# FebriantiW/Homomorphic-Encryption-and-Federated-Learning-based-Privacy-Preserving-CNN-Training-

Measured on AMD Instinct MI355X. Metric: fl_rounds_per_sec, higher is better.
Workload: dtype bf16; 1 GPU; model=cnn2, image=28x28x1, global_batch=32, local_epochs=10, samples_per_client=720, augment=none, parallelism=fl-dp1 (1 GPU = 1 client), device=cuda

## Files before the change

### hefl/csrc/bindings.cpp

```cpp
#include <torch/extension.h>

#include <vector>

void ntt_batch(torch::Tensor x, torch::Tensor w, torch::Tensor wsh, int64_t q);
void intt_batch(torch::Tensor x, torch::Tensor winv, torch::Tensor winvsh,
                int64_t q, int64_t ninv, int64_t ninvsh);
torch::Tensor modmul(torch::Tensor a, torch::Tensor b, int64_t q);
torch::Tensor modmul_scalar(torch::Tensor a, int64_t s, int64_t q);
torch::Tensor modadd(torch::Tensor a, torch::Tensor b, int64_t q);
torch::Tensor modsub(torch::Tensor a, torch::Tensor b, int64_t q);
void modreduce_(torch::Tensor x, torch::Tensor qs);
torch::Tensor cbd21(torch::Tensor bits);
void ntt_limbs(torch::Tensor x, torch::Tensor w, torch::Tensor wsh,
               torch::Tensor qs, int64_t L);
void intt_limbs(torch::Tensor x, torch::Tensor winv, torch::Tensor winvsh,
                torch::Tensor qs, torch::Tensor ninv, torch::Tensor ninvsh,
                int64_t L);
torch::Tensor modmul_limbs(torch::Tensor a, torch::Tensor b, torch::Tensor qs,
                           torch::Tensor ratios, int64_t L, int64_t n);
torch::Tensor modmul_scalar_limbs(torch::Tensor a, torch::Tensor scalars,
                                  torch::Tensor shoups, torch::Tensor qs,
                                  int64_t L, int64_t n);
torch::Tensor modadd_limbs(torch::Tensor a, torch::Tensor b, torch::Tensor qs,
                           int64_t L, int64_t n);
torch::Tensor modadd3_limbs(torch::Tensor a, torch::Tensor b, torch::Tensor c,
                            torch::Tensor qs, int64_t L, int64_t n);
torch::Tensor modsub_limbs(torch::Tensor a, torch::Tensor b, torch::Tensor qs,
                           int64_t L, int64_t aL, int64_t n);
torch::Tensor bcast_center_mod(torch::Tensor x, int64_t qc, torch::Tensor qs,
                               torch::Tensor ratios, int64_t L);
std::vector<torch::Tensor> ct_mul(torch::Tensor a, torch::Tensor b,
                                  torch::Tensor qs, torch::Tensor ratios,
                                  int64_t L, int64_t n);
std::vector<torch::Tensor> ks_inner(torch::Tensor dig, torch::Tensor rlk,
                                    torch::Tensor qs, torch::Tensor ratios,
                                    int64_t D, int64_t Lp, int64_t n);
torch::Tensor uniform_center_rns(torch::Tensor bits, int64_t smudge_bits,
                                 torch::Tensor qs, torch::Tensor ratios,
                                 int64_t L);
torch::Tensor pdec_share(torch::Tensor ct, torch::Tensor s_hat,
                         torch::Tensor e_hat, bool add_c0, torch::Tensor qs,
                         torch::Tensor ratios);
torch::Tensor galois_lift(torch::Tensor c, int64_t ginv, torch::Tensor qs,
                          torch::Tensor ratios);
torch::Tensor galois_perm_add(torch::Tensor ct, torch::Tensor ks0,
                              torch::Tensor ks1, torch::Tensor perm,
                              torch::Tensor qs);

torch::Tensor fft_encode(torch::Tensor vals, torch::Tensor tw_enc,
                         double scale);
torch::Tensor fft_decode(torch::Tensor coeffs, torch::Tensor tw_dec,
                         double scale, int64_t k);

torch::Tensor conv2d_fwd(torch::Tensor x, torch::Tensor w, torch::Tensor b,
                         int64_t stride, bool relu, int64_t pad);
torch::Tensor conv2d_dgrad(torch::Tensor dy, torch::Tensor w, int64_t stride,
                           int64_t H, int64_t W, int64_t pad);
torch::Tensor conv2d_wgrad(torch::Tensor dy, torch::Tensor x, int64_t stride,
                           int64_t R, int64_t S, int64_t pad, int64_t gkey);
torch::Tensor linear_fwd(torch::Tensor x, torch::Tensor w, torch::Tensor b,
                         bool relu);
torch::Tensor linear_dgrad(torch::Tensor dy, torch::Tensor w);
torch::Tensor linear_wgrad(torch::Tensor dy, torch::Tensor x);
std::vector<torch::Tensor> maxpool2x2_fwd(torch::Tensor x);
torch::Tensor synth_batch(torch::Tensor templates, torch::Tensor labels,
                          int64_t seed, double zoom, double shear,
                          int64_t flip);
torch::Tensor synth_batch_g(torch::Tensor templates, torch::Tensor labels,
                            torch::Tensor seed_buf, int64_t salt, double zoom,
                            double shear, int64_t flip);
torch::Tensor maxpool2x2_bwd(torch::Tensor dy, torch::Tensor idx, int64_t H,
                             int64_t W);
std::vector<torch::Tensor> softmax_xent_fwd(torch::Tensor logits,
                                            torch::Tensor labels,
                                            torch::Tensor acc_loss,
                                            torch::Tensor acc_correct);
torch::Tensor softmax_xent_bwd(torch::Tensor probs, torch::Tensor labels,
                               torch::Tensor dloss, bool out_bf16);
void fused_adam(torch::Tensor p, torch::Tensor g, torch::Tensor m,
                torch::Tensor v, double lr, double b1, double b2, double eps,
                double bc1, double bc2);
void adam_prep(torch::Tensor step, torch::Tensor sched, torch::Tensor hyper,
               double b1, double b2);
torch::Tensor relu_bwd(torch::Tensor dy, torch::Tensor y);
std::vector<torch::Tensor> bn_fwd(torch::Tensor x, torch::Tensor gamma,
                                  torch::Tensor beta, torch::Tensor rmean,
                                  torch::Tensor rvar, double eps,
                                  double momentum, bool relu,
                                  torch::Tensor sums);
torch::Tensor bn_apply(torch::Tensor x, torch::Tensor mean,
                       torch::Tensor invstd, torch::Tensor gamma,
                       torch::Tensor beta, bool relu);
std::vector<torch::Tensor> bn_bwd(torch::Tensor dy, torch::Tensor x,
                                  torch::Tensor mean, torch::Tensor invstd,
                                  torch::Tensor gamma, bool train,
                                  torch::Tensor relu_y, torch::Tensor fwd_sums);
std::vector<torch::Tensor> maxpool_fwd(torch::Tensor x, int64_t k, int64_t s,
// ... 51 lines not shown
    m.def("cbd21", &cbd21, "centered binomial eta=21 from 64-bit draws");
    m.def("ntt_limbs", &ntt_limbs, "fused multi-limb forward NTT [R, L, n]");
    m.def("intt_limbs", &intt_limbs, "fused multi-limb inverse NTT");
    m.def("modmul_limbs", &modmul_limbs);
    m.def("modmul_scalar_limbs", &modmul_scalar_limbs);
    m.def("modadd_limbs", &modadd_limbs, "per-limb modular add over [.., L, n]");
    m.def("modadd3_limbs", &modadd3_limbs, "fused 3-way per-limb modular add");
    m.def("modsub_limbs", &modsub_limbs, "per-limb modular sub over [.., L, n]");
    m.def("bcast_center_mod", &bcast_center_mod,
          "[.., n] -> [.., L, n] center + per-limb Barrett reduce");
    m.def("ct_mul", &ct_mul, "fused ct x ct tensor product (d0, d1, d2)");
    m.def("ks_inner", &ks_inner, "fused key-switch digit inner product");
    m.def("uniform_center_rns", &uniform_center_rns,
          "64-bit draws [.., n] -> smudging noise residues [.., L, n]");
    m.def("pdec_share", &pdec_share,
          "threshold decryption share c1*s + e (+ c0) over [.., 2, L, n]");
    m.def("galois_lift", &galois_lift,
          "X -> X^g on key-switch digits [.., D, n], lifted to [.., D, Lp, n]");
    m.def("galois_perm_add", &galois_perm_add,
          "rotated ciphertext (c0[perm] + ks0, ks1) over [.., 2, L, n]");
    m.def("fft_encode", &fft_encode,
          "CKKS special-FFT encode: f64 slots -> int64 coeffs");
    m.def("fft_decode", &fft_decode,
          "CKKS special-FFT decode: int64 coeffs -> f32 slots");
    m.def("conv2d_fwd", &conv2d_fwd);
    m.def("conv2d_dgrad", &conv2d_dgrad);
    m.def("conv2d_wgrad", &conv2d_wgrad, py::arg("dy"), py::arg("x"),
          py::arg("stride"), py::arg("R"), py::arg("S"), py::arg("pad"),
          py::arg("gkey") = 0);
    m.def("linear_fwd", &linear_fwd);
    m.def("linear_dgrad", &linear_dgrad);
    m.def("linear_wgrad", &linear_wgrad);
    m.def("maxpool2x2_fwd", &maxpool2x2_fwd);
    m.def("synth_batch", &synth_batch, py::arg("templates"), py::arg("labels"),
          py::arg("seed"), py::arg("zoom") = 0.0, py::arg("shear") = 0.0,
          py::arg("flip") = 0);
    m.def("synth_batch_g", &synth_batch_g, py::arg("templates"),
          py::arg("labels"), py::arg("seed_buf"), py::arg("salt"),
          py::arg("zoom") = 0.0, py::arg("shear") = 0.0, py::arg("flip") = 0);
    m.def("maxpool2x2_bwd", &maxpool2x2_bwd);
    m.def("softmax_xent_fwd", &softmax_xent_fwd);
    m.def("softmax_xent_bwd", &softmax_xent_bwd);
    m.def("fused_adam", &fused_adam);
    m.def("adam_prep", &adam_prep);
    m.def("relu_bwd", &relu_bwd);
    m.def("bn_fwd", &bn_fwd);
    m.def("bn_apply", &bn_apply);
    m.def("bn_bwd", &bn_bwd);
    m.def("maxpool_fwd", &maxpool_fwd);
    m.def("maxpool_bwd", &maxpool_bwd);
    m.def("avgpool_global_fwd", &avgpool_global_fwd);
    m.def("avgpool_global_bwd", &avgpool_global_bwd);
    m.def("add_relu", &add_relu);
    m.def("bias_grad", &bias_grad, py::arg("dy"), py::arg("gkey") = 0);
    m.def("relu_bias_bwd", &relu_bias_bwd, py::arg("dy"), py::arg("y"),
          py::arg("gkey") = 0);
    m.def("pool_relu_bias_bwd", &pool_relu_bias_bwd, py::arg("dy"),
          py::arg("idx"), py::arg("p"), py::arg("H"), py::arg("W"),
          py::arg("gkey") = 0);
    m.def("fused_adam_mt", &fused_adam_mt);
    m.def("pad_channels", &pad_channels,
          "zero-pad NHWC channel dim to C8 (stem -> glds MFMA path)");
    m.def("dense_head2_fwd", &dense_head2_fwd);
    m.def("dense_head2_bwd", &dense_head2_bwd,
          "single-launch backward of the 2-layer dense head (M <= 32)");
    m.def("linear_bwd_pair", &linear_bwd_pair,
// ... 10 lines not shown
```

### hefl/csrc/cnn.hip

```cpp

#include <hip/hip_runtime.h>
#include <hip/hip_bf16.h>
#include <torch/extension.h>
#include <ATen/cuda/CUDAContext.h>

#include <algorithm>
#include <unordered_map>

#define CHECK_GPU(x) TORCH_CHECK((x).is_cuda(), #x " must be on GPU")

namespace {

using bf16_t = __bf16;
typedef bf16_t bf16x8 __attribute__((ext_vector_type(8)));
typedef float f32x4 __attribute__((ext_vector_type(4)));
typedef unsigned short u16x8 __attribute__((ext_vector_type(8)));

__device__ __forceinline__ float bf2f(unsigned short u) {
    union { unsigned int i; float f; } v;
    v.i = ((unsigned int)u) << 16;
    return v.f;
}

__device__ __forceinline__ unsigned short f2bf(float f) {
    union { float f; unsigned int i; } v;
    v.f = f;
    unsigned int x = v.i;
    unsigned int lsb = (x >> 16) & 1;
    x += 0x7fffu + lsb;
    if ((v.i & 0x7fffffffu) > 0x7f800000u) return 0x7fc0u;
    return (unsigned short)(x >> 16);
}


constexpr int BM = 64;
constexpr int BN = 16;
constexpr int BK = 32;
constexpr int TPB = 256;

// ... 128 lines not shown

template <int BM, int BN, int WM, int WN, int FM, int FN>
__device__ __forceinline__ void tile_mfma(
    const unsigned short (&As)[BM][32], const unsigned short (&Bs)[BN][32],
    f32x4 (&acc)[FM][FN], int wave, int lane) {
    const int wm = wave / WN, wn = wave % WN;
    const int half = lane >> 4, sub = lane & 15;
    bf16x8 a[FM], b[FN];
#pragma unroll
    for (int i = 0; i < FM; ++i)
        a[i] = *reinterpret_cast<const bf16x8*>(
            &As[wm * FM * 16 + i * 16 + sub][half * 8]);
#pragma unroll
    for (int j = 0; j < FN; ++j)
        b[j] = *reinterpret_cast<const bf16x8*>(
            &Bs[wn * FN * 16 + j * 16 + sub][half * 8]);
#pragma unroll
    for (int i = 0; i < FM; ++i)
#pragma unroll
        for (int j = 0; j < FN; ++j)
            acc[i][j] = __builtin_amdgcn_mfma_f32_16x16x32_bf16(a[i], b[j],
                                                                acc[i][j], 0, 0, 0);
}

__device__ __forceinline__ void copy16(unsigned short* dst,
                                       const unsigned short* src) {
    *reinterpret_cast<uint4*>(dst) = *reinterpret_cast<const uint4*>(src);
}

__device__ __forceinline__ void zero16(unsigned short* dst) {
    *reinterpret_cast<uint4*>(dst) = uint4{0, 0, 0, 0};
}

template <int BM, int BN, int WM, int WN, int FM, int FN>
__global__ void __launch_bounds__(TPB)
conv_fwd_kernel(const unsigned short* __restrict__ x,
                const unsigned short* __restrict__ w,
                const float* __restrict__ bias, unsigned short* __restrict__ y,
                ConvShape s, int relu) {
    __shared__ ConvTile<BM, BN, WM, WN, FM, FN> sm;
    constexpr int RPT = BM * 4 / TPB;
    const int tid = threadIdx.x;
    const int wave = tid >> 6;
    const int lane = tid & 63;
    const int m0 = blockIdx.x * BM;
    const int n0 = blockIdx.y * BN;
    const int M = s.N * s.OH * s.OW;
    const int KK = s.R * s.S * s.C;
    const bool fast = (s.C % 8 == 0);

    int arows[RPT], am_[RPT], a_n[RPT], a_oh[RPT], a_ow[RPT];
    const int akc = (tid & 3) * 8;
#pragma unroll
    for (int t = 0; t < RPT; ++t) {
        arows[t] = (tid + t * TPB) >> 2;
        const int am = m0 + arows[t];
        am_[t] = am;
        a_n[t] = a_oh[t] = a_ow[t] = 0;
        if (am < M) {
            a_n[t] = am / (s.OH * s.OW);
            int rem = am % (s.OH * s.OW);
            a_oh[t] = rem / s.OW;
            a_ow[t] = rem % s.OW;
        }
    }

    f32x4 acc[FM][FN];
#pragma unroll
    for (int i = 0; i < FM; ++i)
#pragma unroll
        for (int j = 0; j < FN; ++j) acc[i][j] = f32x4{0.f, 0.f, 0.f, 0.f};

    for (int k0 = 0; k0 < KK; k0 += 32) {
#pragma unroll
        for (int t = 0; t < RPT; ++t) {
            const int k = k0 + akc;
            unsigned short* dst = &sm.As[arows[t]][akc];
            if (am_[t] < M && k < KK) {
                if (fast) {
                    int rs = (int)fdiv((unsigned)k, s.fC), c = k - rs * s.C;
                    int r = (int)fdiv((unsigned)rs, s.fS), ss = rs - r * s.S;
                    int ih = a_oh[t] * s.stride + r - s.pad;
                    int iw = a_ow[t] * s.stride + ss - s.pad;
                    if (ih >= 0 && ih < s.H && iw >= 0 && iw < s.W)
                        copy16(dst, x + ((((int64_t)a_n[t] * s.H + ih) * s.W + iw)
                                             * s.C + c));
                    else
                        zero16(dst);
                } else {
#pragma unroll
                    for (int j = 0; j < 8; ++j) {
                        int kk = k + j;
                        unsigned short v = 0;
                        if (kk < KK) {
                            int rs = (int)fdiv((unsigned)kk, s.fC);
                            int c = kk - rs * s.C;
// ... 8 lines not shown
                    }
                }
            } else {
                zero16(dst);
            }
        }
        for (int i = tid; i < BN * 4; i += TPB) {
            const int col = i >> 2;
            const int kc = (i & 3) * 8;
            const int ko = n0 + col, k = k0 + kc;
            unsigned short* dst = &sm.Bs[col][kc];
            if (ko < s.Kout && k < KK) {
                if ((KK & 7) == 0) {
                    copy16(dst, w + (int64_t)ko * KK + k);
                } else {
#pragma unroll
                    for (int j = 0; j < 8; ++j)
                        dst[j] = (k + j < KK) ? w[(int64_t)ko * KK + k + j] : 0;
                }
            } else {
                zero16(dst);
            }
        }
        __syncthreads();
        tile_mfma<BM, BN, WM, WN, FM, FN>(sm.As, sm.Bs, acc, wave, lane);
        __syncthreads();
    }
    const int wm = wave / WN, wn = wave % WN;
#pragma unroll
    for (int j = 0; j < FN; ++j) {
        const int col = n0 + wn * FN * 16 + j * 16 + (lane & 15);
        if (col >= s.Kout) continue;
        const float bv = bias ? bias[col] : 0.f;
#pragma unroll
        for (int i = 0; i < FM; ++i)
#pragma unroll
            for (int r = 0; r < 4; ++r) {
                int row = m0 + wm * FM * 16 + i * 16 + (lane >> 4) * 4 + r;
                if (row >= M) continue;
                float v = acc[i][j][r] + bv;
                if (relu) v = v > 0.f ? v : 0.f;
                y[(int64_t)row * s.Kout + col] = f2bf(v);
            }
    }
}


typedef uint32_t __attribute__((address_space(3))) lds_u32_t;
typedef const uint32_t __attribute__((address_space(1))) glb_u32_t;

__device__ __forceinline__ int xcd_remap(int wg, int nwg) {
    if (nwg < 16) return wg;
    const int xcd = wg & 7;
    const int q = nwg >> 3, r = nwg & 7;
    const int base = xcd < r ? xcd * (q + 1) : r * (q + 1) + (xcd - r) * q;
    return base + (wg >> 3);
}

__device__ __forceinline__ void glds16(const unsigned short* src, void* lds_base) {
    __builtin_amdgcn_global_load_lds((glb_u32_t*)src, (lds_u32_t*)lds_base, 16,
                                     0, 0);
}

template <int BM, int BN, int WM, int WN, int FM, int FN, int BK = 32>
__global__ void __launch_bounds__(TPB)
conv_fwd_glds_kernel(const unsigned short* __restrict__ x,
                     const unsigned short* __restrict__ w,
                     const float* __restrict__ bias,
                     unsigned short* __restrict__ y,
                     float* __restrict__ y32,
                     const unsigned short* __restrict__ zbuf, ConvShape s,
                     int relu, int k_chunks) {
    __shared__ unsigned short smem[3 * (BM + BN) * BK];
    auto As = [&](int buf) -> unsigned short (*)[BK] {
        return reinterpret_cast<unsigned short(*)[BK]>(smem + buf * (BM + BN) * BK);
    };
    auto Bs = [&](int buf) -> unsigned short (*)[BK] {
        return reinterpret_cast<unsigned short(*)[BK]>(smem + buf * (BM + BN) * BK
                                                       + BM * BK);
    };
    constexpr int RPT = BM * (BK / 8) / TPB;
    constexpr int BPT = BN * (BK / 8) / TPB;
    const int tid = threadIdx.x;
    const int wave = tid >> 6;
    const int lane = tid & 63;
    const int m0 = xcd_remap(blockIdx.x, gridDim.x) * BM;
    const int n0 = blockIdx.y * BN;
    const int M = s.N * s.OH * s.OW;
    const int KK = s.R * s.S * s.C;

    constexpr int CPR = BK / 8;
    int a_n[RPT], a_oh[RPT], a_ow[RPT];
    int akcs[RPT], arow3[RPT];
    bool a_ok[RPT];
#pragma unroll
    for (int t = 0; t < RPT; ++t) {
        const int arow = (tid + t * TPB) / CPR;
        arow3[t] = (arow >> 2) & 3;
        akcs[t] = ((tid % CPR) ^ (CPR == 4 ? arow3[t] : 0)) * 8;
        const int am = m0 + arow;
        a_ok[t] = am < M;
        a_n[t] = a_oh[t] = a_ow[t] = 0;
        if (a_ok[t]) {
            a_n[t] = am / (s.OH * s.OW);
            int rem = am % (s.OH * s.OW);
            a_oh[t] = rem / s.OW;
            a_ow[t] = rem % s.OW;
        }
    }

    auto stage = [&](int buf, int k0) {
#pragma unroll
        for (int t = 0; t < RPT; ++t) {
            const int k = k0 + akcs[t];
            const unsigned short* src = zbuf;
            if (a_ok[t] && k < KK) {
                int rs = (int)fdiv((unsigned)k, s.fC), c = k - rs * s.C;
                int r = (int)fdiv((unsigned)rs, s.fS), ss = rs - r * s.S;
                int ih = a_oh[t] * s.stride + r - s.pad;
                int iw = a_ow[t] * s.stride + ss - s.pad;
                if (ih >= 0 && ih < s.H && iw >= 0 && iw < s.W)
                    src = x + ((((int64_t)a_n[t] * s.H + ih) * s.W + iw) * s.C
                               + c);
            }
            char* base = (char*)&As(buf)[0][0] + (wave + t * 4) * 1024;
            glds16(src, base);
        }
#pragma unroll
        for (int t = 0; t < BPT; ++t) {
            const int i = tid + t * TPB;
            const int korow = i / CPR;
            const int ko = n0 + korow;
            const int kc = ((i % CPR) ^ (CPR == 4 ? ((korow >> 2) & 3) : 0)) * 8;
            const int k = k0 + kc;
            const unsigned short* src = zbuf;
            if (ko < s.Kout && k < KK) src = w + (int64_t)ko * KK + k;
            char* base = (char*)&Bs(buf)[0][0] + (wave + t * 4) * 1024;
            glds16(src, base);
        }
    };
// ... 22 lines not shown
            const int wm = wave / WN, wn = wave % WN;
            const int half = lane >> 4, sub = lane & 15;
            const int swz = (BK == 32) ? ((sub >> 2) & 3) : 0;
#pragma unroll
            for (int kk = 0; kk < BK; kk += 32) {
                bf16x8 a[FM], b[FN];
#pragma unroll
                for (int i = 0; i < FM; ++i)
                    a[i] = *reinterpret_cast<const bf16x8*>(
                        &As(buf)[wm * FM * 16 + i * 16 + sub]
                                [kk + ((half ^ swz) * 8)]);
#pragma unroll
                for (int j = 0; j < FN; ++j)
                    b[j] = *reinterpret_cast<const bf16x8*>(
                        &Bs(buf)[wn * FN * 16 + j * 16 + sub]
                                [kk + ((half ^ swz) * 8)]);
#pragma unroll
                for (int i = 0; i < FM; ++i)
#pragma unroll
                    for (int j = 0; j < FN; ++j)
                        acc[i][j] = __builtin_amdgcn_mfma_f32_16x16x32_bf16(
                            a[i], b[j], acc[i][j], 0, 0, 0);
            }
        }
        buf = buf == 2 ? 0 : buf + 1;
    }
    asm volatile("s_waitcnt vmcnt(0)" ::: "memory");
    const int wm = wave / WN, wn = wave % WN;
#pragma unroll
    for (int j = 0; j < FN; ++j) {
        const int col = n0 + wn * FN * 16 + j * 16 + (lane & 15);
        if (col >= s.Kout) continue;
        const float bv = bias ? bias[col] : 0.f;
#pragma unroll
        for (int i = 0; i < FM; ++i)
#pragma unroll
            for (int r = 0; r < 4; ++r) {
                int row = m0 + wm * FM * 16 + i * 16 + (lane >> 4) * 4 + r;
                if (row >= M) continue;
                if (k_chunks > 1) {
                    atomicAdd(y32 + (int64_t)row * s.Kout + col, acc[i][j][r]);
                } else {
                    float v = acc[i][j][r] + bv;
                    if (relu) v = v > 0.f ? v : 0.f;
                    y[(int64_t)row * s.Kout + col] = f2bf(v);
                }
            }
    }
}


__device__ __forceinline__ int swz128(int byte_off) {
    return byte_off ^ (((byte_off >> 9) & 1) << 5);
}

template <int BM, int BN, int WM, int WN, int FM, int FN, bool PAD0>
__global__ void __launch_bounds__(TPB)
conv_fwd_glds64_kernel(const unsigned short* __restrict__ x,
                       const unsigned short* __restrict__ w,
                       const float* __restrict__ bias,
                       unsigned short* __restrict__ y,
                       float* __restrict__ y32,
                       const unsigned short* __restrict__ zbuf, ConvShape s,
                       int relu, int k_chunks) {
    constexpr int BK = 64;
    constexpr int NW = TPB / 64;
    static_assert(WM * WN == NW, "wave grid must cover the block");
    static_assert(BM == WM * FM * 16 && BN == WN * FN * 16, "tile mismatch");
    constexpr int ABYTES = BM * BK * 2;
    constexpr int RPT = (BM * BK / 8) / TPB;
    constexpr int BPT = (BN * BK / 8) / TPB;
    static_assert(RPT * TPB * 8 == BM * BK && BPT * TPB * 8 == BN * BK);
    __shared__ unsigned short smem[2 * (BM + BN) * BK];
    const int tid = threadIdx.x;
    const int wave = tid >> 6;
    const int lane = tid & 63;
    const int m0 = blockIdx.x * BM;
    const int n0 = blockIdx.y * BN;
    const int M = s.N * s.OH * s.OW;
    const int KK = s.R * s.S * s.C;
// ... 2938 lines not shown
        }
        (void)hipMemsetAsync(p, 0, numel * sizeof(float), stream);
        it = bufs.emplace(key, std::make_pair(p, numel)).first;
    }
    if (it->second.second != numel) {
        ok = false;
        return {};
    }
    ok = true;
    return torch::from_blob(it->second.first, sizes,
                            opts.dtype(torch::kFloat32));
}

float* acc_pool(int64_t n, const torch::TensorOptions& opts,
                hipStream_t stream, torch::Tensor& holder) {
    static torch::Tensor pool;
    auto f32 = opts.dtype(torch::kFloat32);
    if (!pool.defined() || pool.device() != f32.device_opt().value() ||
        pool.numel() < n) {
        hipStreamCaptureStatus st = hipStreamCaptureStatusNone;
        (void)hipStreamIsCapturing(stream, &st);
        if (st != hipStreamCaptureStatusNone) {
            holder = torch::zeros({n}, f32);
            return holder.data_ptr<float>();
        }
        pool = torch::zeros({n}, f32);
    }
    return pool.data_ptr<float>();
}

}


torch::Tensor conv2d_fwd(torch::Tensor x, torch::Tensor w, torch::Tensor b,
                         int64_t stride, bool relu, int64_t pad) {
    CHECK_GPU(x);
    TORCH_CHECK(x.is_contiguous() && w.is_contiguous());
    TORCH_CHECK(x.dtype() == torch::kBFloat16 && w.dtype() == torch::kBFloat16);
    ConvShape s = make_shape(x, w, (int)stride, (int)pad);
    auto y = torch::empty({s.N, s.OH, s.OW, s.Kout}, x.options());
    const int M = s.N * s.OH * s.OW;
    const float* bias = b.numel() ? b.data_ptr<float>() : nullptr;
    auto stream = at::cuda::getCurrentCUDAStream();
    const int KKf = s.R * s.S * s.C;
    const char* t3env = getenv("HEFL_TILE3");
    const int t3mode = t3env ? t3env[0] - '0' : 1;
    if (t3mode != 0 && s.R == 3 && s.S == 3 && s.stride == 1 && s.pad <= 1 &&
        s.C % 32 == 0 && s.Kout > 16 &&
        (t3mode >= 2 || s.Kout <= 32)) {
        const int BN3 = (t3mode == 3 || s.Kout <= 32) ? 32 : 64;
        const int kt = ceildiv(s.Kout, BN3);
        const int64_t min_tiles = t3mode == 2 ? 1 : 256;
        auto tiles = [&](int th, int tw) {
            return (int64_t)s.N * ceildiv(s.OH, th) * ceildiv(s.OW, tw) * kt;
        };
        int TH = 0;
        if (s.OH >= 12 && tiles(16, 16) >= min_tiles) TH = 16;
        else if (t3mode >= 2 && s.OH >= 6 && tiles(8, 16) >= min_tiles) TH = 8;
        if (TH) {
            const int th_ = ceildiv(s.OH, TH), tw_ = ceildiv(s.OW, 16);
            dim3 grid((unsigned)(s.N * th_ * tw_), (unsigned)kt);
            #define LAUNCH_T3(TH_, TW_, BN_, WM_, WN_, FM_, FN_)              \
                hipLaunchKernelGGL(                                           \
                    (conv_fwd_tile3_kernel<TH_, TW_, BN_, WM_, WN_, FM_,      \
                                           FN_>),                             \
                    grid, dim3(TPB), 0, stream, bf_ptr(x), bf_ptr(w), bias,   \
                    bf_ptr_mut(y), s, relu ? 1 : 0, th_, tw_)
            if (TH == 16 && BN3 == 64)      LAUNCH_T3(16, 16, 64, 2, 2, 8, 2);
            else if (TH == 16)              LAUNCH_T3(16, 16, 32, 4, 1, 4, 2);
            else if (BN3 == 64)             LAUNCH_T3(8, 16, 64, 2, 2, 4, 2);
            else                            LAUNCH_T3(8, 16, 32, 2, 2, 4, 1);
            #undef LAUNCH_T3
            return y;
        }
    }
    static const bool use64 = [] {
        const char* e = getenv("HEFL_GLDS64");
        return e && e[0] == '1';
    }();
    if (use64 && s.Kout > 16 && s.C % 8 == 0 && KKf % 8 == 0) {
        static torch::Tensor zbuf64;
        if (!zbuf64.defined() || zbuf64.device() != x.device())
            zbuf64 = torch::zeros({8}, x.options());
        const bool narrow = s.Kout <= 32;
        const int BM = narrow ? 256 : 128, BN = narrow ? 32 : 64;
        int tiles = ceildiv(M, BM) * ceildiv(s.Kout, BN);
        int ksteps = ceildiv(KKf, 64);
        int k_chunks = 1;
        if (tiles < 256 && ksteps >= 8)
            k_chunks = std::max(1, std::min(ksteps / 2, 512 / std::max(tiles, 1)));
        dim3 grid(ceildiv(M, BM), ceildiv(s.Kout, BN), k_chunks);
        torch::Tensor y32;
        float* y32p = nullptr;
        if (k_chunks > 1)
            y32p = acc_pool((int64_t)M * s.Kout, x.options(), stream, y32);
        #define LAUNCH_F64(BM_, BN_, WM_, WN_, FM_, FN_, P0)                  \
            hipLaunchKernelGGL((conv_fwd_glds64_kernel<BM_, BN_, WM_, WN_,    \
                                                       FM_, FN_, P0>),       \
                               grid, dim3(TPB), 0, stream, bf_ptr(x),         \
                               bf_ptr(w), bias, bf_ptr_mut(y), y32p,          \
                               bf_ptr(zbuf64), s, relu ? 1 : 0, k_chunks)
        if (narrow) {
            if (s.pad == 0) LAUNCH_F64(256, 32, 4, 1, 4, 2, true);
            else            LAUNCH_F64(256, 32, 4, 1, 4, 2, false);
        } else {
            if (s.pad == 0) LAUNCH_F64(128, 64, 2, 2, 4, 2, true);
            else            LAUNCH_F64(128, 64, 2, 2, 4, 2, false);
        }
        #undef LAUNCH_F64
        if (k_chunks > 1) {
            int64_t total = (int64_t)M * s.Kout;
            hipLaunchKernelGGL(linear_epilogue_kernel,
                               dim3((int)std::min<int64_t>(ceildiv(total, 256), 2048)),
                               dim3(256), 0, stream, y32p, bias,
                               bf_ptr_mut(y), total, s.Kout, relu ? 1 : 0, 1, 1);
        }
        return y;
    }
    if (s.Kout > 16 && s.C % 8 == 0 && KKf % 8 == 0) {
        static torch::Tensor zbuf;
        if (!zbuf.defined() || zbuf.device() != x.device())
            zbuf = torch::zeros({8}, x.options());
        int tiles = ceildiv(M, 64) * ceildiv(s.Kout, 64);
        int ksteps = ceildiv(KKf, 32);
        int k_chunks = 1;
        if (tiles < 256 && ksteps >= 16)
            k_chunks = std::max(1, std::min(ksteps / 4, 512 / tiles));
        dim3 grid(ceildiv(M, 64), ceildiv(s.Kout, 64), k_chunks);
        if (k_chunks > 1) {
            torch::Tensor y32h;
            float* y32p = acc_pool((int64_t)M * s.Kout, x.options(), stream,
                                   y32h);
            hipLaunchKernelGGL((conv_fwd_glds_kernel<64, 64, 2, 2, 2, 2, 32>),
                               grid, dim3(TPB), 0, stream, bf_ptr(x), bf_ptr(w),
                               bias, bf_ptr_mut(y), y32p,
                               bf_ptr(zbuf), s, relu ? 1 : 0, k_chunks);
            int64_t total = (int64_t)M * s.Kout;
            hipLaunchKernelGGL(linear_epilogue_kernel,
                               dim3((int)std::min<int64_t>(ceildiv(total, 256), 2048)),
                               dim3(256), 0, stream, y32p, bias,
                               bf_ptr_mut(y), total, s.Kout, relu ? 1 : 0, 1, 1);
        } else {
            hipLaunchKernelGGL((conv_fwd_glds_kernel<64, 64, 2, 2, 2, 2, 32>),
                               grid, dim3(TPB), 0, stream, bf_ptr(x), bf_ptr(w),
                               bias, bf_ptr_mut(y), (float*)nullptr,
                               bf_ptr(zbuf), s, relu ? 1 : 0, 1);
        }
    } else if (s.Kout > 16) {
        dim3 grid(ceildiv(M, 64), ceildiv(s.Kout, 64));
        hipLaunchKernelGGL((conv_fwd_kernel<64, 64, 2, 2, 2, 2>), grid,
                           dim3(TPB), 0, stream, bf_ptr(x), bf_ptr(w), bias,
                           bf_ptr_mut(y), s, relu ? 1 : 0);
    } else {
        dim3 grid(ceildiv(M, 64), ceildiv(s.Kout, 16));
        hipLaunchKernelGGL((conv_fwd_kernel<64, 16, 4, 1, 1, 1>), grid,
                           dim3(TPB), 0, stream, bf_ptr(x), bf_ptr(w), bias,
                           bf_ptr_mut(y), s, relu ? 1 : 0);
    }
    return y;
}

torch::Tensor conv2d_dgrad(torch::Tensor dy, torch::Tensor w, int64_t stride,
                           int64_t H, int64_t W, int64_t pad) {
    CHECK_GPU(dy);
    TORCH_CHECK(dy.is_contiguous() && w.is_contiguous());
    const int N = (int)dy.size(0);
    const int C = (int)w.size(3);
    ConvShape s;
    s.N = N; s.H = (int)H; s.W = (int)W; s.C = C;
    s.Kout = (int)w.size(0); s.R = (int)w.size(1); s.S = (int)w.size(2);
    s.stride = (int)stride; s.pad = (int)pad;
    s.OH = (int)dy.size(1); s.OW = (int)dy.size(2);
    fill_magic(s);
    auto dx = torch::empty({N, (int64_t)H, (int64_t)W, C}, dy.options());
    const int M = N * (int)H * (int)W;
    auto stream = at::cuda::getCurrentCUDAStream();
    const char* t3env_d = getenv("HEFL_TILE3");
    const int t3mode_d = t3env_d ? t3env_d[0] - '0' : 1;
    if (t3mode_d != 0 && s.R == 3 && s.S == 3 && stride == 1 && pad <= 1 &&
        s.Kout % 32 == 0 && C > 16 && (t3mode_d == 2 || C <= 32)) {
        ConvShape s3;
        s3.N = N; s3.H = s.OH; s3.W = s.OW; s3.C = s.Kout;
        s3.Kout = C; s3.R = 3; s3.S = 3; s3.stride = 1; s3.pad = 2 - (int)pad;
        s3.OH = (int)H; s3.OW = (int)W;
        fill_magic(s3);
        const int BN3 = C <= 32 ? 32 : 64;
        const int kt = ceildiv(C, BN3);
        const int64_t min_tiles = t3mode_d == 2 ? 1 : 256;
        const int64_t t16 = (int64_t)N * ceildiv(s3.OH, 16)
                            * ceildiv(s3.OW, 16) * kt;
        if (s3.OH >= 12 && t16 >= min_tiles) {
            auto wT = torch::empty({C, 3, 3, s.Kout}, w.options());
// ... 968 lines not shown
```

### hefl/ops/functional.py

```python
from __future__ import annotations

import torch
import torch.nn.functional as F

import hefl


def _C():
    return hefl.load_extension()


def _gpu_dtype(t: torch.Tensor) -> torch.Tensor:
    sh = getattr(t, "_bf16", None)
    if sh is not None:
        return sh
    return t if t.dtype == torch.bfloat16 else t.to(torch.bfloat16)


def _want_cpad(C: int, Kout: int) -> bool:
    return C % 8 != 0 and Kout > 16 and Kout % 8 == 0


def _pad8(t: torch.Tensor) -> torch.Tensor:
    C = t.shape[-1]
    return _C().pad_channels(t.contiguous(), ((C + 7) // 8) * 8)


import os

_BN_ATOMIC_MODE = os.getenv("HEFL_BN_ATOMIC", "0")

_BWD_FORK = os.getenv("HEFL_BWD_FORK", "0") == "1"
_SIDE_STREAMS = {}


def _fork_side(dev):
    s = _SIDE_STREAMS.get(dev)
    if s is None:
        s = torch.cuda.Stream(device=dev)
        _SIDE_STREAMS[dev] = s
    return s

_HEAD_XENT = os.getenv("HEFL_HEAD_XENT", "1") != "0"
_LIN_PAIR = os.getenv("HEFL_LIN_PAIR", "1") != "0"

GRAPH_NO_ZERO = False



class _Conv2dFn(torch.autograd.Function):
    @staticmethod
    def forward(ctx, x, w, b, stride: int, relu: bool, pad: int):
        ctx.stride = stride
        ctx.relu = relu
        ctx.pad = pad
        ctx.has_bias = b is not None
        ctx.cpad = False
        ctx.wkey = id(w)
        ctx.bkey = id(b) if b is not None else 0
        if x.is_cuda:
            wb = _gpu_dtype(w)
            if _want_cpad(x.shape[-1], w.shape[0]):
                ctx.cpad = True
                ctx.in_C = x.shape[-1]
                x = _pad8(x)
                wb = _pad8(wb)
            bb = b.detach().float() if b is not None else torch.empty(0, device=x.device)
            y = _C().conv2d_fwd(x.contiguous(), wb.contiguous(), bb, stride, relu, pad)
            ctx.save_for_backward(x, wb, y)
        else:
            xf = x.float()
            xn = xf.permute(0, 3, 1, 2)
            wn = w.permute(0, 3, 1, 2)
            yn = F.conv2d(xn, wn, b, stride=stride, padding=pad)
            y = yn.permute(0, 2, 3, 1).contiguous()
            if relu:
                y = F.relu(y)
# ... 84 lines not shown
        return y

    @staticmethod
    def backward(ctx, dy):
        (idx,) = ctx.saved_tensors
        N, H, W, C = ctx.in_shape
        if dy.is_cuda:
            dx = _C().maxpool2x2_bwd(dy.contiguous(), idx, H, W)
        else:
            dyn = dy.float().permute(0, 3, 1, 2)
            dxn = F.max_unpool2d(dyn, idx, 2, 2, output_size=(H, W))
            dx = dxn.permute(0, 2, 3, 1).contiguous()
        return dx


def maxpool2x2(x):
    return _MaxPool2x2Fn.apply(x)


class _ConvReluPoolFn(torch.autograd.Function):

    @staticmethod
    def forward(ctx, x, w, b, pad: int):
        ctx.pad = pad
        ctx.wkey = id(w)
        ctx.bkey = id(b)
        wb = _gpu_dtype(w)
        ctx.cpad = _want_cpad(x.shape[-1], w.shape[0])
        if ctx.cpad:
            ctx.in_C = x.shape[-1]
            x = _pad8(x)
            wb = _pad8(wb)
        bb = b.detach().float()
        y = _C().conv2d_fwd(x.contiguous(), wb.contiguous(), bb, 1, True, pad)
        ctx.conv_hw = (y.shape[1], y.shape[2])
        p, idx = _C().maxpool2x2_fwd(y)
        ctx.save_for_backward(x, wb, p, idx)
        return p

    @staticmethod
    def backward(ctx, dy):
        x, w, p, idx = ctx.saved_tensors
        ch, cw = ctx.conv_hw
        bkey = ctx.bkey if GRAPH_NO_ZERO else 0
        dym, db = _C().pool_relu_bias_bwd(dy.contiguous(), idx, p, ch, cw,
                                          gkey=bkey)
        wg = ctx.wkey if (GRAPH_NO_ZERO and not ctx.cpad) else 0
        fork = (_BWD_FORK and ctx.needs_input_grad[0]
                and torch.cuda.is_current_stream_capturing())
        if fork:
            cur = torch.cuda.current_stream()
            side = _fork_side(dy.device)
            ev = torch.cuda.Event()
            ev.record(cur)
            with torch.cuda.stream(side):
                side.wait_event(ev)
                dw = _C().conv2d_wgrad(dym, x.contiguous(), 1, w.shape[1],
                                       w.shape[2], ctx.pad, gkey=wg)
                if ctx.cpad:
                    dw = dw[..., :ctx.in_C].contiguous()
                ev2 = torch.cuda.Event()
                ev2.record(side)
            dx = _C().conv2d_dgrad(dym, w, 1, x.shape[1], x.shape[2], ctx.pad)
            cur.wait_event(ev2)
        else:
            dx = _C().conv2d_dgrad(dym, w, 1, x.shape[1], x.shape[2],
                                   ctx.pad) \
                if ctx.needs_input_grad[0] else None
            dw = _C().conv2d_wgrad(dym, x.contiguous(), 1, w.shape[1],
# ... 384 lines not shown
```

Baseline: 48.00 rounds/s.

## Fuse 2x2 maxpool into conv forward epilogue via pool-ordered GEMM rows

Adds a POOL template mode to the gather and GLDS conv forward kernels. GEMM rows are reordered so that each group of four consecutive rows is one 2x2 pooling window, which lets each MFMA lane's four accumulator rows be pooled in registers after bias and ReLU. The kernel then writes only the pooled output and the argmax index. This removes the full-size conv activation write, the separate maxpool kernel launch and its read. The conv-forward dispatch logic is factored into a plan struct, and shapes that pick the tile3, GLDS64 or split-K paths fall back to conv followed by a separate pool. Odd output dimensions drop the last row or column, which matches floor pooling.

```diff
diff --git a/hefl/csrc/bindings.cpp b/hefl/csrc/bindings.cpp
--- a/hefl/csrc/bindings.cpp
+++ b/hefl/csrc/bindings.cpp
@@ -1,5 +1,6 @@
 #include <torch/extension.h>
 
+#include <tuple>
 #include <vector>
 
 void ntt_batch(torch::Tensor x, torch::Tensor w, torch::Tensor wsh, int64_t q);
@@ -63,6 +64,9 @@
 torch::Tensor linear_dgrad(torch::Tensor dy, torch::Tensor w);
 torch::Tensor linear_wgrad(torch::Tensor dy, torch::Tensor x);
 std::vector<torch::Tensor> maxpool2x2_fwd(torch::Tensor x);
+std::tuple<torch::Tensor, torch::Tensor, int64_t, int64_t>
+conv2d_relu_pool_fwd(torch::Tensor x, torch::Tensor w, torch::Tensor b,
+                     int64_t pad);
 torch::Tensor synth_batch(torch::Tensor templates, torch::Tensor labels,
                           int64_t seed, double zoom, double shear,
                           int64_t flip);
@@ -180,6 +184,7 @@
     m.def("linear_dgrad", &linear_dgrad);
     m.def("linear_wgrad", &linear_wgrad);
     m.def("maxpool2x2_fwd", &maxpool2x2_fwd);
+    m.def("conv2d_relu_pool_fwd", &conv2d_relu_pool_fwd);
     m.def("synth_batch", &synth_batch, py::arg("templates"), py::arg("labels"),
           py::arg("seed"), py::arg("zoom") = 0.0, py::arg("shear") = 0.0,
           py::arg("flip") = 0);
diff --git a/hefl/csrc/cnn.hip b/hefl/csrc/cnn.hip
--- a/hefl/csrc/cnn.hip
+++ b/hefl/csrc/cnn.hip
@@ -5,6 +5,7 @@
 #include <ATen/cuda/CUDAContext.h>
 
 #include <algorithm>
+#include <tuple>
 #include <unordered_map>
 
 #define CHECK_GPU(x) TORCH_CHECK((x).is_cuda(), #x " must be on GPU")
@@ -199,12 +200,45 @@
     *reinterpret_cast<uint4*>(dst) = uint4{0, 0, 0, 0};
 }
 
-template <int BM, int BN, int WM, int WN, int FM, int FN>
+
+__device__ __forceinline__ void pool_row_decode(int am, int PH, int PW, int& n,
+                                                int& oh, int& ow) {
+    const int win = am >> 2, q = am & 3;
+    n = win / (PH * PW);
+    const int rem = win % (PH * PW);
+    const int ph = rem / PW;
+    oh = 2 * ph + (q >> 1);
+    ow = 2 * (rem - ph * PW) + (q & 1);
+}
+
+__device__ __forceinline__ void pool_epilogue_store(
+    f32x4 acc, float bv, unsigned short* __restrict__ p,
+    uint8_t* __restrict__ pidx, int64_t o) {
+    unsigned short u[4];
+#pragma unroll
+    for (int r = 0; r < 4; ++r) {
+        float v = acc[r] + bv;
+        u[r] = f2bf(v > 0.f ? v : 0.f);
+    }
+    unsigned short bu = u[0];
+    float best = bf2f(u[0]);
+    int bi = 0;
+#pragma unroll
+    for (int r = 1; r < 4; ++r) {
+        const float v = bf2f(u[r]);
+        if (v > best) { best = v; bu = u[r]; bi = r; }
+    }
+    p[o] = bu;
+    pidx[o] = (uint8_t)bi;
+}
+
+template <int BM, int BN, int WM, int WN, int FM, int FN, bool POOL = false>
 __global__ void __launch_bounds__(TPB)
 conv_fwd_kernel(const unsigned short* __restrict__ x,
                 const unsigned short* __restrict__ w,
                 const float* __restrict__ bias, unsigned short* __restrict__ y,
-                ConvShape s, int relu) {
+                uint8_t* __restrict__ pidx, ConvShape s, int relu) {
+    static_assert(!POOL || (BM % 4 == 0), "pool windows must not straddle tiles");
     __shared__ ConvTile<BM, BN, WM, WN, FM, FN> sm;
     constexpr int RPT = BM * 4 / TPB;
     const int tid = threadIdx.x;
@@ -212,7 +246,8 @@
     const int lane = tid & 63;
     const int m0 = blockIdx.x * BM;
     const int n0 = blockIdx.y * BN;
-    const int M = s.N * s.OH * s.OW;
+    const int PH = s.OH >> 1, PW = s.OW >> 1;
+    const int M = POOL ? s.N * PH * PW * 4 : s.N * s.OH * s.OW;
     const int KK = s.R * s.S * s.C;
     const bool fast = (s.C % 8 == 0);
 
@@ -225,10 +260,14 @@
         am_[t] = am;
         a_n[t] = a_oh[t] = a_ow[t] = 0;
         if (am < M) {
-            a_n[t] = am / (s.OH * s.OW);
-            int rem = am % (s.OH * s.OW);
-            a_oh[t] = rem / s.OW;
-            a_ow[t] = rem % s.OW;
+            if constexpr (POOL) {
+                pool_row_decode(am, PH, PW, a_n[t], a_oh[t], a_ow[t]);
+            } else {
+                a_n[t] = am / (s.OH * s.OW);
+                int rem = am % (s.OH * s.OW);
+                a_oh[t] = rem / s.OW;
+                a_ow[t] = rem % s.OW;
+            }
         }
     }
 
@@ -303,6 +342,15 @@
         const int col = n0 + wn * FN * 16 + j * 16 + (lane & 15);
         if (col >= s.Kout) continue;
         const float bv = bias ? bias[col] : 0.f;
+        if constexpr (POOL) {
+#pragma unroll
+            for (int i = 0; i < FM; ++i) {
+                const int row = m0 + wm * FM * 16 + i * 16 + (lane >> 4) * 4;
+                if (row >= M) continue;
+                pool_epilogue_store(acc[i][j], bv, y, pidx,
+                                    (int64_t)(row >> 2) * s.Kout + col);
+            }
+        } else {
 #pragma unroll
         for (int i = 0; i < FM; ++i)
 #pragma unroll
@@ -313,6 +361,7 @@
                 if (relu) v = v > 0.f ? v : 0.f;
                 y[(int64_t)row * s.Kout + col] = f2bf(v);
             }
+        }
     }
 }
 
@@ -333,15 +382,18 @@
                                      0, 0);
 }
 
-template <int BM, int BN, int WM, int WN, int FM, int FN, int BK = 32>
+template <int BM, int BN, int WM, int WN, int FM, int FN, int BK = 32,
+          bool POOL = false>
 __global__ void __launch_bounds__(TPB)
 conv_fwd_glds_kernel(const unsigned short* __restrict__ x,
                      const unsigned short* __restrict__ w,
                      const float* __restrict__ bias,
                      unsigned short* __restrict__ y,
                      float* __restrict__ y32,
+                     uint8_t* __restrict__ pidx,
                      const unsigned short* __restrict__ zbuf, ConvShape s,
                      int relu, int k_chunks) {
+    static_assert(!POOL || (BM % 4 == 0), "pool windows must not straddle tiles");
     __shared__ unsigned short smem[3 * (BM + BN) * BK];
     auto As = [&](int buf) -> unsigned short (*)[BK] {
         return reinterpret_cast<unsigned short(*)[BK]>(smem + buf * (BM + BN) * BK);
@@ -357,7 +409,8 @@
     const int lane = tid & 63;
     const int m0 = xcd_remap(blockIdx.x, gridDim.x) * BM;
     const int n0 = blockIdx.y * BN;
-    const int M = s.N * s.OH * s.OW;
+    const int PH = s.OH >> 1, PW = s.OW >> 1;
+    const int M = POOL ? s.N * PH * PW * 4 : s.N * s.OH * s.OW;
     const int KK = s.R * s.S * s.C;
 
     constexpr int CPR = BK / 8;
@@ -373,10 +426,14 @@
         a_ok[t] = am < M;
         a_n[t] = a_oh[t] = a_ow[t] = 0;
         if (a_ok[t]) {
-            a_n[t] = am / (s.OH * s.OW);
-            int rem = am % (s.OH * s.OW);
-            a_oh[t] = rem / s.OW;
-            a_ow[t] = rem % s.OW;
+            if constexpr (POOL) {
+                pool_row_decode(am, PH, PW, a_n[t], a_oh[t], a_ow[t]);
+            } else {
+                a_n[t] = am / (s.OH * s.OW);
+                int rem = am % (s.OH * s.OW);
+                a_oh[t] = rem / s.OW;
+                a_ow[t] = rem % s.OW;
+            }
         }
     }
 
@@ -465,6 +522,15 @@
         const int col = n0 + wn * FN * 16 + j * 16 + (lane & 15);
         if (col >= s.Kout) continue;
         const float bv = bias ? bias[col] : 0.f;
+        if constexpr (POOL) {
+#pragma unroll
+            for (int i = 0; i < FM; ++i) {
+                const int row = m0 + wm * FM * 16 + i * 16 + (lane >> 4) * 4;
+                if (row >= M) continue;
+                pool_epilogue_store(acc[i][j], bv, y, pidx,
+                                    (int64_t)(row >> 2) * s.Kout + col);
+            }
+        } else {
 #pragma unroll
         for (int i = 0; i < FM; ++i)
 #pragma unroll
@@ -479,6 +545,7 @@
                     y[(int64_t)row * s.Kout + col] = f2bf(v);
                 }
             }
+        }
     }
 }
 
@@ -3483,16 +3550,15 @@
 }
 
 
-torch::Tensor conv2d_fwd(torch::Tensor x, torch::Tensor w, torch::Tensor b,
-                         int64_t stride, bool relu, int64_t pad) {
-    CHECK_GPU(x);
-    TORCH_CHECK(x.is_contiguous() && w.is_contiguous());
-    TORCH_CHECK(x.dtype() == torch::kBFloat16 && w.dtype() == torch::kBFloat16);
-    ConvShape s = make_shape(x, w, (int)stride, (int)pad);
-    auto y = torch::empty({s.N, s.OH, s.OW, s.Kout}, x.options());
+struct ConvFwdPlan {
+    enum Kind { TILE3, GLDS64, GLDS32, GATHER64, GATHER16 } kind;
+    int k_chunks = 1;
+    int TH = 0, BN3 = 0;
+};
+
+static ConvFwdPlan conv_fwd_plan(const ConvShape& s) {
+    ConvFwdPlan p;
     const int M = s.N * s.OH * s.OW;
-    const float* bias = b.numel() ? b.data_ptr<float>() : nullptr;
-    auto stream = at::cuda::getCurrentCUDAStream();
     const int KKf = s.R * s.S * s.C;
     const char* t3env = getenv("HEFL_TILE3");
     const int t3mode = t3env ? t3env[0] - '0' : 1;
@@ -3509,37 +3575,75 @@
         if (s.OH >= 12 && tiles(16, 16) >= min_tiles) TH = 16;
         else if (t3mode >= 2 && s.OH >= 6 && tiles(8, 16) >= min_tiles) TH = 8;
         if (TH) {
-            const int th_ = ceildiv(s.OH, TH), tw_ = ceildiv(s.OW, 16);
-            dim3 grid((unsigned)(s.N * th_ * tw_), (unsigned)kt);
-            #define LAUNCH_T3(TH_, TW_, BN_, WM_, WN_, FM_, FN_)              \
-                hipLaunchKernelGGL(                                           \
-                    (conv_fwd_tile3_kernel<TH_, TW_, BN_, WM_, WN_, FM_,      \
-                                           FN_>),                             \
-                    grid, dim3(TPB), 0, stream, bf_ptr(x), bf_ptr(w), bias,   \
-                    bf_ptr_mut(y), s, relu ? 1 : 0, th_, tw_)
-            if (TH == 16 && BN3 == 64)      LAUNCH_T3(16, 16, 64, 2, 2, 8, 2);
-            else if (TH == 16)              LAUNCH_T3(16, 16, 32, 4, 1, 4, 2);
-            else if (BN3 == 64)             LAUNCH_T3(8, 16, 64, 2, 2, 4, 2);
-            else                            LAUNCH_T3(8, 16, 32, 2, 2, 4, 1);
-            #undef LAUNCH_T3
-            return y;
+            p.kind = ConvFwdPlan::TILE3;
+            p.TH = TH;
+            p.BN3 = BN3;
+            return p;
         }
     }
     static const bool use64 = [] {
         const char* e = getenv("HEFL_GLDS64");
         return e && e[0] == '1';
     }();
-    if (use64 && s.Kout > 16 && s.C % 8 == 0 && KKf % 8 == 0) {
-        static torch::Tensor zbuf64;
-        if (!zbuf64.defined() || zbuf64.device() != x.device())
-            zbuf64 = torch::zeros({8}, x.options());
+    const bool glds_ok = s.Kout > 16 && s.C % 8 == 0 && KKf % 8 == 0;
+    if (use64 && glds_ok) {
+        p.kind = ConvFwdPlan::GLDS64;
         const bool narrow = s.Kout <= 32;
         const int BM = narrow ? 256 : 128, BN = narrow ? 32 : 64;
-        int tiles = ceildiv(M, BM) * ceildiv(s.Kout, BN);
-        int ksteps = ceildiv(KKf, 64);
-        int k_chunks = 1;
+        const int tiles = ceildiv(M, BM) * ceildiv(s.Kout, BN);
+        const int ksteps = ceildiv(KKf, 64);
         if (tiles < 256 && ksteps >= 8)
-            k_chunks = std::max(1, std::min(ksteps / 2, 512 / std::max(tiles, 1)));
+            p.k_chunks = std::max(1, std::min(ksteps / 2, 512 / std::max(tiles, 1)));
+    } else if (glds_ok) {
+        p.kind = ConvFwdPlan::GLDS32;
+        const int tiles = ceildiv(M, 64) * ceildiv(s.Kout, 64);
+        const int ksteps = ceildiv(KKf, 32);
+        if (tiles < 256 && ksteps >= 16)
+            p.k_chunks = std::max(1, std::min(ksteps / 4, 512 / tiles));
+    } else {
+        p.kind = s.Kout > 16 ? ConvFwdPlan::GATHER64 : ConvFwdPlan::GATHER16;
+    }
+    return p;
+}
+
+static const unsigned short* conv_zbuf(const torch::Tensor& x) {
+    static torch::Tensor zbuf;
+    if (!zbuf.defined() || zbuf.device() != x.device())
+        zbuf = torch::zeros({8}, x.options());
+    return bf_ptr(zbuf);
+}
+
+torch::Tensor conv2d_fwd(torch::Tensor x, torch::Tensor w, torch::Tensor b,
+                         int64_t stride, bool relu, int64_t pad) {
+    CHECK_GPU(x);
+    TORCH_CHECK(x.is_contiguous() && w.is_contiguous());
+    TORCH_CHECK(x.dtype() == torch::kBFloat16 && w.dtype() == torch::kBFloat16);
+    ConvShape s = make_shape(x, w, (int)stride, (int)pad);
+    auto y = torch::empty({s.N, s.OH, s.OW, s.Kout}, x.options());
+    const int M = s.N * s.OH * s.OW;
+    const float* bias = b.numel() ? b.data_ptr<float>() : nullptr;
+    auto stream = at::cuda::getCurrentCUDAStream();
+    const ConvFwdPlan plan = conv_fwd_plan(s);
+    const int k_chunks = plan.k_chunks;
+    if (plan.kind == ConvFwdPlan::TILE3) {
+        const int TH = plan.TH, BN3 = plan.BN3;
+        const int kt = ceildiv(s.Kout, BN3);
+        const int th_ = ceildiv(s.OH, TH), tw_ = ceildiv(s.OW, 16);
+        dim3 grid((unsigned)(s.N * th_ * tw_), (unsigned)kt);
+        #define LAUNCH_T3(TH_, TW_, BN_, WM_, WN_, FM_, FN_)                  \
+            hipLaunchKernelGGL(                                               \
+                (conv_fwd_tile3_kernel<TH_, TW_, BN_, WM_, WN_, FM_, FN_>),   \
+                grid, dim3(TPB), 0, stream, bf_ptr(x), bf_ptr(w), bias,       \
+                bf_ptr_mut(y), s, relu ? 1 : 0, th_, tw_)
+        if (TH == 16 && BN3 == 64)      LAUNCH_T3(16, 16, 64, 2, 2, 8, 2);
+        else if (TH == 16)              LAUNCH_T3(16, 16, 32, 4, 1, 4, 2);
+        else if (BN3 == 64)             LAUNCH_T3(8, 16, 64, 2, 2, 4, 2);
+        else                            LAUNCH_T3(8, 16, 32, 2, 2, 4, 1);
+        #undef LAUNCH_T3
+    } else if (plan.kind == ConvFwdPlan::GLDS64) {
+        const bool narrow = s.Kout <= 32;
+        const int BM = narrow ? 256 : 128, BN = narrow ? 32 : 64;
+        const unsigned short* zbuf = conv_zbuf(x);
         dim3 grid(ceildiv(M, BM), ceildiv(s.Kout, BN), k_chunks);
         torch::Tensor y32;
         float* y32p = nullptr;
@@ -3550,7 +3654,7 @@
                                                        FM_, FN_, P0>),       \
                                grid, dim3(TPB), 0, stream, bf_ptr(x),         \
                                bf_ptr(w), bias, bf_ptr_mut(y), y32p,          \
-                               bf_ptr(zbuf64), s, relu ? 1 : 0, k_chunks)
+                               zbuf, s, relu ? 1 : 0, k_chunks)
         if (narrow) {
             if (s.pad == 0) LAUNCH_F64(256, 32, 4, 1, 4, 2, true);
             else            LAUNCH_F64(256, 32, 4, 1, 4, 2, false);
@@ -3566,17 +3670,8 @@
                                dim3(256), 0, stream, y32p, bias,
                                bf_ptr_mut(y), total, s.Kout, relu ? 1 : 0, 1, 1);
         }
-        return y;
-    }
-    if (s.Kout > 16 && s.C % 8 == 0 && KKf % 8 == 0) {
-        static torch::Tensor zbuf;
-        if (!zbuf.defined() || zbuf.device() != x.device())
-            zbuf = torch::zeros({8}, x.options());
-        int tiles = ceildiv(M, 64) * ceildiv(s.Kout, 64);
-        int ksteps = ceildiv(KKf, 32);
-        int k_chunks = 1;
-        if (tiles < 256 && ksteps >= 16)
-            k_chunks = std::max(1, std::min(ksteps / 4, 512 / tiles));
+    } else if (plan.kind == ConvFwdPlan::GLDS32) {
+        const unsigned short* zbuf = conv_zbuf(x);
         dim3 grid(ceildiv(M, 64), ceildiv(s.Kout, 64), k_chunks);
         if (k_chunks > 1) {
             torch::Tensor y32h;
@@ -3584,8 +3679,8 @@
                                    y32h);
             hipLaunchKernelGGL((conv_fwd_glds_kernel<64, 64, 2, 2, 2, 2, 32>),
                                grid, dim3(TPB), 0, stream, bf_ptr(x), bf_ptr(w),
-                               bias, bf_ptr_mut(y), y32p,
-                               bf_ptr(zbuf), s, relu ? 1 : 0, k_chunks);
+                               bias, bf_ptr_mut(y), y32p, (uint8_t*)nullptr,
+                               zbuf, s, relu ? 1 : 0, k_chunks);
             int64_t total = (int64_t)M * s.Kout;
             hipLaunchKernelGGL(linear_epilogue_kernel,
                                dim3((int)std::min<int64_t>(ceildiv(total, 256), 2048)),
@@ -3595,20 +3690,67 @@
             hipLaunchKernelGGL((conv_fwd_glds_kernel<64, 64, 2, 2, 2, 2, 32>),
                                grid, dim3(TPB), 0, stream, bf_ptr(x), bf_ptr(w),
                                bias, bf_ptr_mut(y), (float*)nullptr,
-                               bf_ptr(zbuf), s, relu ? 1 : 0, 1);
-        }
-    } else if (s.Kout > 16) {
+                               (uint8_t*)nullptr, zbuf, s, relu ? 1 : 0, 1);
+        }
+    } else if (plan.kind == ConvFwdPlan::GATHER64) {
         dim3 grid(ceildiv(M, 64), ceildiv(s.Kout, 64));
         hipLaunchKernelGGL((conv_fwd_kernel<64, 64, 2, 2, 2, 2>), grid,
                            dim3(TPB), 0, stream, bf_ptr(x), bf_ptr(w), bias,
-                           bf_ptr_mut(y), s, relu ? 1 : 0);
+                           bf_ptr_mut(y), (uint8_t*)nullptr, s, relu ? 1 : 0);
     } else {
         dim3 grid(ceildiv(M, 64), ceildiv(s.Kout, 16));
         hipLaunchKernelGGL((conv_fwd_kernel<64, 16, 4, 1, 1, 1>), grid,
                            dim3(TPB), 0, stream, bf_ptr(x), bf_ptr(w), bias,
-                           bf_ptr_mut(y), s, relu ? 1 : 0);
+                           bf_ptr_mut(y), (uint8_t*)nullptr, s, relu ? 1 : 0);
     }
     return y;
+}
+
+std::vector<torch::Tensor> maxpool2x2_fwd(torch::Tensor x);
+
+std::tuple<torch::Tensor, torch::Tensor, int64_t, int64_t>
+conv2d_relu_pool_fwd(torch::Tensor x, torch::Tensor w, torch::Tensor b,
+                     int64_t pad) {
+    CHECK_GPU(x);
+    TORCH_CHECK(x.is_contiguous() && w.is_contiguous());
+    TORCH_CHECK(x.dtype() == torch::kBFloat16 && w.dtype() == torch::kBFloat16);
+    ConvShape s = make_shape(x, w, 1, (int)pad);
+    const int PH = s.OH / 2, PW = s.OW / 2;
+    const ConvFwdPlan plan = conv_fwd_plan(s);
+    const bool fuse =
+        PH > 0 && PW > 0 &&
+        (plan.kind == ConvFwdPlan::GATHER16 ||
+         plan.kind == ConvFwdPlan::GATHER64 ||
+         (plan.kind == ConvFwdPlan::GLDS32 && plan.k_chunks == 1));
+    if (!fuse) {
+        auto y = conv2d_fwd(x, w, b, 1, true, pad);
+        auto pi = maxpool2x2_fwd(y);
+        return {pi[0], pi[1], (int64_t)s.OH, (int64_t)s.OW};
+    }
+    auto p = torch::empty({s.N, PH, PW, s.Kout}, x.options());
+    auto idx = torch::empty({s.N, PH, PW, s.Kout},
+                            x.options().dtype(torch::kUInt8));
+    const int M = s.N * PH * PW * 4;
+    const float* bias = b.numel() ? b.data_ptr<float>() : nullptr;
+    auto stream = at::cuda::getCurrentCUDAStream();
+    if (plan.kind == ConvFwdPlan::GLDS32) {
+        dim3 grid(ceildiv(M, 64), ceildiv(s.Kout, 64), 1);
+        hipLaunchKernelGGL(
+            (conv_fwd_glds_kernel<64, 64, 2, 2, 2, 2, 32, true>), grid,
+            dim3(TPB), 0, stream, bf_ptr(x), bf_ptr(w), bias, bf_ptr_mut(p),
+            (float*)nullptr, idx.data_ptr<uint8_t>(), conv_zbuf(x), s, 1, 1);
+    } else if (plan.kind == ConvFwdPlan::GATHER64) {
+        dim3 grid(ceildiv(M, 64), ceildiv(s.Kout, 64));
+        hipLaunchKernelGGL((conv_fwd_kernel<64, 64, 2, 2, 2, 2, true>), grid,
+                           dim3(TPB), 0, stream, bf_ptr(x), bf_ptr(w), bias,
+                           bf_ptr_mut(p), idx.data_ptr<uint8_t>(), s, 1);
+    } else {
+        dim3 grid(ceildiv(M, 64), ceildiv(s.Kout, 16));
+        hipLaunchKernelGGL((conv_fwd_kernel<64, 16, 4, 1, 1, 1, true>), grid,
+                           dim3(TPB), 0, stream, bf_ptr(x), bf_ptr(w), bias,
+                           bf_ptr_mut(p), idx.data_ptr<uint8_t>(), s, 1);
+    }
+    return {p, idx, (int64_t)s.OH, (int64_t)s.OW};
 }
 
 torch::Tensor conv2d_dgrad(torch::Tensor dy, torch::Tensor w, int64_t stride,
diff --git a/hefl/ops/functional.py b/hefl/ops/functional.py
--- a/hefl/ops/functional.py
+++ b/hefl/ops/functional.py
@@ -43,6 +43,7 @@
 
 _HEAD_XENT = os.getenv("HEFL_HEAD_XENT", "1") != "0"
 _LIN_PAIR = os.getenv("HEFL_LIN_PAIR", "1") != "0"
+_CONV_POOL = os.getenv("HEFL_CONV_POOL", "1") != "0"
 
 GRAPH_NO_ZERO = False
 
@@ -193,9 +194,15 @@
             x = _pad8(x)
             wb = _pad8(wb)
         bb = b.detach().float()
-        y = _C().conv2d_fwd(x.contiguous(), wb.contiguous(), bb, 1, True, pad)
-        ctx.conv_hw = (y.shape[1], y.shape[2])
-        p, idx = _C().maxpool2x2_fwd(y)
+        if _CONV_POOL:
+            p, idx, ch, cw = _C().conv2d_relu_pool_fwd(
+                x.contiguous(), wb.contiguous(), bb, pad)
+            ctx.conv_hw = (ch, cw)
+        else:
+            y = _C().conv2d_fwd(x.contiguous(), wb.contiguous(), bb, 1, True,
+                                pad)
+            ctx.conv_hw = (y.shape[1], y.shape[2])
+            p, idx = _C().maxpool2x2_fwd(y)
         ctx.save_for_backward(x, wb, p, idx)
         return p
 
```

Measured after the change: 51.64 rounds/s (median of 6 runs). 7.6% higher.
